# AdrianoEttari/DiffusionRemoteSensing

Measured on AMD Instinct MI355X. Metric: unet_denoise_steps_per_s, higher is better.
Workload: dtype f16 main + block-scaled fp6 (e2m3) cross terms of tap pairs on the wide 3x3 layers (FL, 11 of 11 launches of the dominant kernel); split bf16 x3 (hi + lo) everywhere else; f32 accumulate

## Files before the change

diffusionremotesensing_amd/csrc/resblock0_sp.hip:

```cpp
#include <stdio.h>
#include <stdlib.h>

#include "conv_epilogue.h"
#include "mfma_policy.h"
#include "sp_sync.h"

namespace {

constexpr int TW_ = 16, TH_ = 8, IW = TW_ + 2, IH = TH_ + 2, NPIX = IW * IH, NBLK_A = (NPIX + 15) / 16;
constexpr int IMG1 = 5 * 4 * 64 * 16, IMG2 = 36 * 32 * 16, IMGS = 4 * 32 * 16, WIN = NPIX * 128;
constexpr int NPOST = 16;
constexpr int XPLANE = (TH_ + 4) * (TW_ + 4) * 16 + 64, XT = 4 * XPLANE;

#ifdef DRS_SP_TIMELINE
__device__ unsigned long long drs_rb0_tl[32];
#define RB_STAMP(i) do { const unsigned long long t_ = __builtin_amdgcn_s_memtime(); tl[i] += t_ - tl_last; tl_last = t_; } while (0)
#else
#define RB_STAMP(i) do { } while (0)
#endif

__global__ __launch_bounds__(512, 1) void resblock0_kernel(ResBlock0Desc d, unsigned w1_gimage, unsigned w2_gimage,
                                                           unsigned ws_gimage) {
  extern __shared__ __attribute__((aligned(16))) char smem[];
  using P = PolicyBF16X3;
  using Frag = typename P::Frag;
  auto mfma = [](const bf16x8& w, const bf16x8& x, const f32x4& c) __attribute__((always_inline)) {
    return __builtin_amdgcn_mfma_f32_16x16x32_bf16(w, x, c, 0, 0, 0);
  };
  const int tid = threadIdx.x, lane = tid & 63, wave = __builtin_amdgcn_readfirstlane(tid >> 6);
  const int lr = lane & 15, kg = lane >> 4;
  char* sW1 = smem;
  char* sW2 = sW1 + 2 * IMG1;
  char* sWs = sW2 + 2 * IMG2;
  char* sWinAll = sWs + 2 * IMGS;
  char* sXAll = sWinAll + 2 * WIN;
  float* sB1 = reinterpret_cast<float*>(sXAll + 2 * XT);
  float* sB2 = sB1 + 64;
  unsigned* sCntRaw = reinterpret_cast<unsigned*>(sB2 + 32);
  float* sPost = sB2 + 32 + 8;
  const int npost = min(d.N, NPOST);
  {
    const char* w1 = reinterpret_cast<const char*>(d.w1);
    for (int i = tid; i < 2 * 20 * 64; i += 512) {
      const int im = i >= 20 * 64, idx = im ? i - 20 * 64 : i;
      const int ch = idx % 64, kgp = (idx / 64) & 3, j = idx / (4 * 64), tap = 2 * j + (kgp >> 1);
      u32x4 v = {0u, 0u, 0u, 0u};
      if (tap < 9) v = *reinterpret_cast<const u32x4*>(w1 + (size_t)im * w1_gimage + ((size_t)(tap * 4 + (kgp & 1)) * 64 + ch) * 16);
      *reinterpret_cast<u32x4*>(sW1 + (size_t)im * IMG1 + (size_t)idx * 16) = v;
    }
    auto copy = [&](char* dst, const char* src, int bytes) __attribute__((always_inline)) {
      for (int o = tid * 16; o < bytes; o += 512 * 16) *reinterpret_cast<u32x4*>(dst + o) = *reinterpret_cast<const u32x4*>(src + o);
    };
    const char* w2 = reinterpret_cast<const char*>(d.w2);
    const char* wsc = reinterpret_cast<const char*>(d.ws);
    copy(sW2, w2, IMG2);
    copy(sW2 + IMG2, w2 + w2_gimage, IMG2);
    copy(sWs, wsc, IMGS);
    copy(sWs + IMGS, wsc + ws_gimage, IMGS);
    for (int i = tid; i < 64; i += 512) sB1[i] = d.b1[i];
    for (int i = tid; i < 32; i += 512) sB2[i] = d.b2[i] + d.bs[i];
    if (tid < 8) sCntRaw[tid] = 0u;
    for (int i = tid; i < npost * 32; i += 512) sPost[i] = d.temb[(size_t)(i >> 5) * d.temb_cs + (i & 31)];
  }
  __syncthreads();

  const int grp = wave >> 2, gw = wave & 3;
  char* sWin = sWinAll + grp * WIN;
  const sp_flag_ptr cWritten = (sp_flag_ptr)(sCntRaw + 2 * grp), cRead = (sp_flag_ptr)(sCntRaw + 2 * grp + 1);
  const int gx = d.W / TW_, gy = d.H / TH_;
  const int total = d.N * gy * gx;
  const int xcd = blockIdx.x & 7, member = blockIdx.x >> 3, members = gridDim.x >> 3;
  const int t_lo = (int)((long long)total * xcd / 8), t_hi = (int)((long long)total * (xcd + 1) / 8);
  const char* zero = reinterpret_cast<const char*>(d.zero_line);
  const char* xb = reinterpret_cast<const char*>(d.x);
  char* sX = sXAll + grp * XT;
  const sp_flag_ptr cTile = (sp_flag_ptr)(sCntRaw + 4 + grp);
  constexpr int XPIX = (TH_ + 4) * (TW_ + 4), XW = TW_ + 4;
  int tx0 = 0, ty0 = 0, n = 0;
  const int qstep_ = 2 * (int)(gridDim.x >> 3);
  const int step_x = qstep_ % gx, step_y = (qstep_ / gx) % gy, step_n = qstep_ / (gx * gy);
  int bx = 0, by = 0;
  auto place_first = [&](int q) __attribute__((always_inline)) {
    bx = q % gx; by = (q / gx) % gy; n = q / (gx * gy);
    tx0 = bx * TW_; ty0 = by * TH_;
  };
  auto place_next = [&]() __attribute__((always_inline)) {
    bx += step_x;
    if (bx >= gx) { bx -= gx; ++by; }
    by += step_y;
    if (by >= gy) { by -= gy; ++n; }
    n += step_n;
    tx0 = bx * TW_; ty0 = by * TH_;
  };
  unsigned goff[4];
#pragma unroll
  for (int i = 0; i < 4; ++i) {
    const int e = i * 256 + gw * 64 + lane, pix = min(e >> 2, XPIX - 1);
    const int py = (pix * 3277) >> 16, px = pix - py * XW;
    goff[i] = (unsigned)((py * d.W + px) * 64 + (e & 3) * 16);
  }
  u32x4 xr[4];
  auto tile_load = [&]() __attribute__((always_inline)) {
    const char* ximg = xb + (size_t)n * d.H * d.W * 64;
    if (ty0 >= 2 && ty0 + TH_ + 2 <= d.H && tx0 >= 2 && tx0 + TW_ + 2 <= d.W) {
      typedef const __attribute__((address_space(1))) char* gptr;
      const unsigned long long gi = (unsigned long long)(ximg + ((long long)(ty0 - 2) * d.W + (tx0 - 2)) * 64);
      gptr g = (gptr)(((unsigned long long)(unsigned)__builtin_amdgcn_readfirstlane((int)(gi >> 32)) << 32) |
                      (unsigned)__builtin_amdgcn_readfirstlane((int)(unsigned)gi));
      asm volatile("" : "+s"(g));
#pragma unroll
      for (int i = 0; i < 4; ++i) xr[i] = *(const __attribute__((address_space(1))) u32x4*)(g + goff[i]);
    } else {
#pragma unroll
      for (int i = 0; i < 4; ++i) {
        const int e = i * 256 + gw * 64 + lane, pix = e >> 2;
        const int py = (pix * 3277) >> 16, px = pix - py * XW;
        const int y = ty0 - 2 + py, x = tx0 - 2 + px;
        const bool ok = pix < XPIX && y >= 0 && y < d.H && x >= 0 && x < d.W;
        xr[i] = *reinterpret_cast<const u32x4*>(ok ? ximg + ((size_t)y * d.W + x) * 64 + (e & 3) * 16 : zero);
      }
    }
  };
  auto tile_store = [&]() __attribute__((always_inline)) {
#pragma unroll
    for (int i = 0; i < 4; ++i) {
      const int e = i * 256 + gw * 64 + lane;
      if ((e >> 2) < XPIX) *reinterpret_cast<u32x4*>(sX + (e & 3) * XPLANE + (e >> 2) * 16) = xr[i];
    }
    sp_release(cTile, lane);
  };
  constexpr int MAXB = NBLK_A / 4;
  static_assert(MAXB * 4 == NBLK_A, "three blocks per wave");
  int wp[MAXB], relL[MAXB], tapL[5];
#pragma unroll
  for (int b = 0; b < MAXB; ++b) {
    const int p = min((gw + 4 * b) * 16 + lr, NPIX - 1);
    const int py = (p * 3641) >> 16, px = p - py * IW;
    wp[b] = p;
    relL[b] = ((py + 1) * XW + px + 1) * 16 + (kg & 1) * XPLANE;
  }
#pragma unroll
  for (int j = 0; j < 5; ++j) {
    const int tap = min(2 * j + (kg >> 1), 8);
    tapL[j] = ((tap / 3 - 1) * XW + tap % 3 - 1) * 16;
  }
  auto operand = [&](int b, int j) __attribute__((always_inline)) {
    const char* p = sX + relL[b] + tapL[j];
    return Frag{*reinterpret_cast<const bf16x8*>(p), *reinterpret_cast<const bf16x8*>(p + 2 * XPLANE)};
  };
  const int q0 = t_lo + 2 * member + grp, qstep = 2 * members;
#ifdef DRS_SP_TIMELINE
  unsigned long long tl[8] = {0, 0, 0, 0, 0, 0, 0, 0};
  const unsigned long long tl_begin = __builtin_amdgcn_s_memtime();
  unsigned long long tl_last = tl_begin, tl_n = 0;
#endif
  if (q0 < t_hi) {
    place_first(q0);
    tile_load();
    tile_store();
    if (q0 + qstep < t_hi) {
      place_next();
      tile_load();
      asm volatile("" :: "v"(xr[0]), "v"(xr[1]), "v"(xr[2]), "v"(xr[3]));
    }
  }
  if (grp == 1) { __builtin_amdgcn_s_sleep(64); __builtin_amdgcn_s_sleep(32); }
  unsigned k = 0;
  u32x4 kept[4] = {};
  int cbx = q0 % gx, cby = (q0 / gx) % gy, cn = q0 / (gx * gy);
  for (int q = q0; q < t_hi; q += qstep, ++k) {
#ifdef DRS_SP_TIMELINE
    ++tl_n;
#endif
    RB_STAMP(7);
    const int cty0 = cby * TH_, ctx0 = cbx * TW_;
    sp_poll_lds(cTile, 4u * (k + 1), d.fault);
    const bool more = q + qstep < t_hi;
    f32x4 acc[MAXB][4];
#pragma unroll
    for (int b = 0; b < MAXB; ++b)
#pragma unroll
      for (int t = 0; t < 4; ++t) acc[b][t] = f32x4{0.f, 0.f, 0.f, 0.f};
    const char* w1lane = sW1 + ((size_t)kg * 64 + lr) * 16;
    Frag a[2][MAXB], wfa[2][2];
#pragma unroll
    for (int b = 0; b < MAXB; ++b) a[0][b] = operand(b, 0);
#pragma unroll
    for (int u = 0; u < 2; ++u) wfa[0][u] = P::load(w1lane, (size_t)IMG1, (size_t)(u * 16) * 16);
#pragma unroll
    for (int st = 0; st < 10; ++st) {
      const int j = st >> 1, h = st & 1;
      if (st + 1 < 10) {
#pragma unroll
        for (int u = 0; u < 2; ++u)
          wfa[(st + 1) & 1][u] = P::load(w1lane, (size_t)IMG1, (size_t)(((st + 1) >> 1) * 4 * 64 + (((st + 1) & 1) * 2 + u) * 16) * 16);
      }
      if (h == 0 && j + 1 < 5) {
#pragma unroll
        for (int b = 0; b < MAXB; ++b) a[(j + 1) & 1][b] = operand(b, j + 1);
      }
      {
        const Frag (&wf)[2] = wfa[st & 1];
#pragma unroll
        for (int u = 0; u < 2; ++u)
#pragma unroll
          for (int b = 0; b < MAXB; ++b) acc[b][2 * h + u] = mfma(wf[u].lo, a[j & 1][b].hi, acc[b][2 * h + u]);
#pragma unroll
        for (int u = 0; u < 2; ++u)
#pragma unroll
          for (int b = 0; b < MAXB; ++b) acc[b][2 * h + u] = mfma(wf[u].hi, a[j & 1][b].lo, acc[b][2 * h + u]);
#pragma unroll
        for (int u = 0; u < 2; ++u)
#pragma unroll
          for (int b = 0; b < MAXB; ++b) acc[b][2 * h + u] = mfma(wf[u].hi, a[j & 1][b].hi, acc[b][2 * h + u]);
      }
      if (h == 0 && j + 1 < 5) __builtin_amdgcn_sched_group_barrier(0x100, 4 + 2 * MAXB, 0);
      else if (st + 1 < 10) __builtin_amdgcn_sched_group_barrier(0x100, 4, 0);
      __builtin_amdgcn_sched_group_barrier(0x008, 18, 0);
      __builtin_amdgcn_sched_barrier(0);
    }
    asm volatile("" :: "v"(kept[0]), "v"(kept[1]), "v"(kept[2]), "v"(kept[3]));
    RB_STAMP(0);
    Frag xs[2];
#pragma unroll
    for (int r = 0; r < 2; ++r) {
      const char* p = sX + ((2 + 2 * gw + r) * XW + 2 + lr) * 16 + (kg & 1) * XPLANE;
      xs[r] = Frag{*reinterpret_cast<const bf16x8*>(p), *reinterpret_cast<const bf16x8*>(p + 2 * XPLANE)};
    }
    float bm[8], bs[8], te[8];
    {
      const float4 m0 = *reinterpret_cast<const float4*>(sB1 + kg * 8), m1 = *reinterpret_cast<const float4*>(sB1 + kg * 8 + 4);
      const float4 s0 = *reinterpret_cast<const float4*>(sB1 + 32 + kg * 8), s1 = *reinterpret_cast<const float4*>(sB1 + 32 + kg * 8 + 4);
      float4 e0, e1;
      if (cn < npost) {
        e0 = *reinterpret_cast<const float4*>(sPost + cn * 32 + kg * 8); e1 = *reinterpret_cast<const float4*>(sPost + cn * 32 + kg * 8 + 4);
      } else {
        const float* gp = d.temb + (size_t)cn * d.temb_cs + kg * 8;
        e0 = *reinterpret_cast<const float4*>(gp); e1 = *reinterpret_cast<const float4*>(gp + 4);
      }
      bm[0] = m0.x; bm[1] = m0.y; bm[2] = m0.z; bm[3] = m0.w; bm[4] = m1.x; bm[5] = m1.y; bm[6] = m1.z; bm[7] = m1.w;
      bs[0] = s0.x; bs[1] = s0.y; bs[2] = s0.z; bs[3] = s0.w; bs[4] = s1.x; bs[5] = s1.y; bs[6] = s1.z; bs[7] = s1.w;
      te[0] = e0.x; te[1] = e0.y; te[2] = e0.z; te[3] = e0.w; te[4] = e1.x; te[5] = e1.y; te[6] = e1.z; te[7] = e1.w;
    }
    RB_STAMP(1);
    sp_poll_lds(cRead, 4u * k, d.fault);
    RB_STAMP(2);
#pragma unroll
    for (int b = 0; b < MAXB; ++b) {
      float v[8];
#pragma unroll
      for (int t = 0; t < 2; ++t)
#pragma unroll
        for (int i = 0; i < 4; ++i)
          v[t * 4 + i] = (drs_maxf(acc[b][t][i] + bm[t * 4 + i], 0.f) + (acc[b][t + 2][i] + bs[t * 4 + i])) + te[t * 4 + i];
      u32x4 hh, hl;
      drs_sp_split8(v, hh, hl);
      int p = wp[b];
      asm volatile("" : "+v"(p));
      const int py = (p * 3641) >> 16, px = p - py * IW;
      const int y = cty0 - 1 + py, x = ctx0 - 1 + px;
      const bool inside = y >= 0 && y < d.H && x >= 0 && x < d.W;
      if (!inside) { hh = u32x4{0u, 0u, 0u, 0u}; hl = u32x4{0u, 0u, 0u, 0u}; }
      if ((gw + 4 * b) * 16 + lr < NPIX) {
        char* wpix = sWin + p * 128;
        const int s0 = ((kg + p) & 7) * 16;
        *reinterpret_cast<u32x4*>(wpix + s0) = hh;
        *reinterpret_cast<u32x4*>(wpix + (s0 ^ 64)) = hl;
      }
    }
    sp_release(cWritten, lane);
    sp_poll_lds(cWritten, 4u * (k + 1), d.fault);
    if (more) tile_store();
    RB_STAMP(3);
    f32x4 o[2][2];
#pragma unroll
    for (int r = 0; r < 2; ++r)
#pragma unroll
      for (int t = 0; t < 2; ++t) o[r][t] = f32x4{0.f, 0.f, 0.f, 0.f};
    const char* w2lane = sW2 + ((size_t)kg * 32 + lr) * 16;
    auto win = [&](int row, int kx) __attribute__((always_inline)) {
      const int p = (2 * gw + row) * IW + lr + kx;
      const char* wpix = sWin + p * 128;
      const int s0 = ((kg + p) & 7) * 16;
      return Frag{*reinterpret_cast<const bf16x8*>(wpix + s0), *reinterpret_cast<const bf16x8*>(wpix + (s0 ^ 64))};
    };
    Frag wr_[4][3];
    auto win_row = [&](int row) __attribute__((always_inline)) {
#pragma unroll
      for (int kx = 0; kx < 3; ++kx) wr_[row][kx] = win(row, kx);
    };
    win_row(0);
    win_row(1);
    {
      const char* wslane = sWs + ((size_t)kg * 32 + lr) * 16;
      Frag wfb[2][2];
      wfb[0][0] = P::load(w2lane, (size_t)IMG2, 0);
      wfb[0][1] = P::load(w2lane, (size_t)IMG2, (size_t)16 * 16);
#pragma unroll
      for (int st = 0; st < 10; ++st) {
#pragma unroll
        for (int t = 0; t < 2; ++t) {
          if (st + 1 < 9) wfb[(st + 1) & 1][t] = P::load(w2lane, (size_t)IMG2, (size_t)((st + 1) * 4 * 32 + t * 16) * 16);
          else if (st + 1 < 10) wfb[(st + 1) & 1][t] = P::load(wslane, (size_t)IMGS, (size_t)(t * 16) * 16);
        }
        if (st == 0) win_row(2);
        if (st == 3) {
          win_row(3);
          sp_release(cRead, lane);
        }
        const int ky = st < 9 ? st / 3 : 0, kx = st < 9 ? st % 3 : 0;
        const Frag& x0f = st < 9 ? wr_[ky][kx] : xs[0];
        const Frag& x1f = st < 9 ? wr_[ky + 1][kx] : xs[1];
        const Frag (&wf)[2] = wfb[st & 1];
#pragma unroll
        for (int t = 0; t < 2; ++t) { o[0][t] = mfma(wf[t].lo, x0f.hi, o[0][t]); o[1][t] = mfma(wf[t].lo, x1f.hi, o[1][t]); }
#pragma unroll
        for (int t = 0; t < 2; ++t) { o[0][t] = mfma(wf[t].hi, x0f.lo, o[0][t]); o[1][t] = mfma(wf[t].hi, x1f.lo, o[1][t]); }
#pragma unroll
        for (int t = 0; t < 2; ++t) { o[0][t] = mfma(wf[t].hi, x0f.hi, o[0][t]); o[1][t] = mfma(wf[t].hi, x1f.hi, o[1][t]); }
        if (st == 0 || st == 3) __builtin_amdgcn_sched_group_barrier(0x100, 10, 0);
        else if (st + 1 < 10) __builtin_amdgcn_sched_group_barrier(0x100, 4, 0);
        __builtin_amdgcn_sched_group_barrier(0x008, 12, 0);
        __builtin_amdgcn_sched_barrier(0);
      }
    }
    if (q + 2 * qstep < t_hi) {
      place_next();
      tile_load();
    }
    RB_STAMP(4);
    {
      const float4 b0 = *reinterpret_cast<const float4*>(sB2 + kg * 8), b1 = *reinterpret_cast<const float4*>(sB2 + kg * 8 + 4);
      const float bb[8] = {b0.x, b0.y, b0.z, b0.w, b1.x, b1.y, b1.z, b1.w};
      const bool lo = lr < 8;
      const size_t pix0 = ((size_t)cn * d.H + cty0 + 2 * gw) * d.W + ctx0 + (lr & 7);
      char* g = reinterpret_cast<char*>(d.out) + pix0 * 128 + (lo ? 0 : 64) + kg * 16;
#pragma unroll
      for (int r = 0; r < 2; ++r) {
        float v[8];
#pragma unroll
        for (int i = 0; i < 4; ++i) { v[i] = drs_maxf(o[r][0][i] + bb[i], 0.f); v[4 + i] = drs_maxf(o[r][1][i] + bb[4 + i], 0.f); }
        u32x4 H, L;
        drs_sp_split8(v, H, L);
        const u32x4 got = drs_dpp_swap8(lo ? L : H);
        kept[2 * r] = lo ? H : got;
        kept[2 * r + 1] = lo ? got : L;
        char* gr = g + (size_t)r * d.W * 128;
        drs_store16(gr, kept[2 * r]);
        drs_store16(gr + 8 * 128, kept[2 * r + 1]);
      }
    }
    RB_STAMP(5);
    cbx += step_x;
    if (cbx >= gx) { cbx -= gx; ++cby; }
    cby += step_y;
    if (cby >= gy) { cby -= gy; ++cn; }
    cn += step_n;
  }
#ifdef DRS_SP_TIMELINE
  if (blockIdx.x == 0 && (wave == 0 || wave == 7) && lane == 0) {
    const int o = wave == 0 ? 0 : 16;
    for (int i = 0; i < 8; ++i) drs_rb0_tl[o + i] = tl[i];
    drs_rb0_tl[o + 8] = tl_n;
    drs_rb0_tl[o + 9] = __builtin_amdgcn_s_memtime() - tl_begin;
  }
#endif
}

size_t resblock0_lds(int N) { return (size_t)2 * (IMG1 + IMG2 + IMGS) + 2 * WIN + 2 * XT + (size_t)(64 + 32 + 8 + 32 * (N < NPOST ? N : NPOST)) * 4; }

}

bool drs_resblock0_supported(int Cin, int Cout, int H, int W) {
  static const bool env = !(getenv("DRS_RB0") && atoi(getenv("DRS_RB0")) == 0);
  return env && Cin == 16 && Cout == 32 && H >= 32 && W >= 32 && H % TH_ == 0 && W % TW_ == 0;
}

int drs_launch_resblock0(const ResBlock0Desc& d, hipStream_t s) {
  DRS_REQUIRE(drs_resblock0_supported(16, 32, d.H, d.W), DRS_ERR_SHAPE, "resblock0: H=%d W=%d", d.H, d.W);
  DRS_REQUIRE(d.x && d.w1 && d.b1 && d.temb && d.w2 && d.b2 && d.ws && d.bs && d.out && d.zero_line, DRS_ERR_ARG, "resblock0: null pointer");
  if (d.N == 0) return DRS_OK;
  int num_cu = 0;
  {
    const int rc = drs_kernel_prepare(reinterpret_cast<const void*>(resblock0_kernel), 160 * 1024, &num_cu);
    if (rc) return rc;
  }
  const unsigned w1_gimage = 9u * 4u * 64u * 16u, w2_gimage = 9u * 4u * 32u * 16u, ws_gimage = 4u * 32u * 16u;
  const int blocks = num_cu / 8 * 8;
  DRS_LAUNCH(resblock0_kernel, dim3((unsigned)blocks), dim3(512), resblock0_lds(d.N), s, d, w1_gimage, w2_gimage, ws_gimage);
  DRS_CHECK_HIP(hipGetLastError());
#ifdef DRS_SP_TIMELINE
  {
    unsigned long long h[32];
    hipEvent_t e0, e1;
    float ms = 0.f;
    DRS_CHECK_HIP(hipEventCreate(&e0)); DRS_CHECK_HIP(hipEventCreate(&e1));
    DRS_CHECK_HIP(hipEventRecord(e0, s));
    DRS_LAUNCH(resblock0_kernel, dim3((unsigned)blocks), dim3(512), resblock0_lds(d.N), s, d, w1_gimage, w2_gimage, ws_gimage);
    DRS_CHECK_HIP(hipEventRecord(e1, s));
    DRS_CHECK_HIP(hipStreamSynchronize(s));
    DRS_CHECK_HIP(hipEventElapsedTime(&ms, e0, e1));
    (void)hipEventDestroy(e0); (void)hipEventDestroy(e1);
    DRS_CHECK_HIP(hipMemcpyFromSymbol(h, HIP_SYMBOL(drs_rb0_tl), sizeof(h)));
    for (int w = 0; w < 2; ++w) {
      const unsigned long long* t = h + 16 * w;
      const double sc = t[8] ? 1.0 / (double)t[8] : 0.0;
      fprintf(stderr, "resblock0 %dx%d wave %d: %.1f us, %llu patches, alive %llu ticks (%.0f / patch) | top %.0f  A-mfma %.0f  A-epi %.0f  bar1 %.0f  "
              "winstore+bar2 %.0f  B-mfma %.0f  B-epi %.0f\n", d.H, d.W, w ? 7 : 0, ms * 1e3, t[8], t[9], t[9] * sc, t[7] * sc, t[0] * sc, t[1] * sc,
              t[2] * sc, t[3] * sc, t[4] * sc, t[5] * sc);
    }
  }
#endif
  return DRS_OK;
}
```

Before: 831.9.

## Overlap first tile loads with LDS weight fill and re-layout input planes

Restructures the resblock0 prologue so each lane issues all global loads for weights, biases and time embedding into registers before writing LDS. The first two input tiles are loaded before the weight fill so their latency overlaps it. Input-tile LDS planes are rearranged with a 64-byte offset on the hi/lo pair to shift bank mapping, and wave-to-group assignment is interleaved. The change also extends timeline instrumentation, and costs extra registers in the prologue.

Result: no change. 838.7 (median of 4 runs) (+0.8%).

```diff
diff --git a/diffusionremotesensing_amd/csrc/resblock0_sp.hip b/diffusionremotesensing_amd/csrc/resblock0_sp.hip
--- a/diffusionremotesensing_amd/csrc/resblock0_sp.hip
+++ b/diffusionremotesensing_amd/csrc/resblock0_sp.hip
@@ -10,10 +10,10 @@
 constexpr int TW_ = 16, TH_ = 8, IW = TW_ + 2, IH = TH_ + 2, NPIX = IW * IH, NBLK_A = (NPIX + 15) / 16;
 constexpr int IMG1 = 5 * 4 * 64 * 16, IMG2 = 36 * 32 * 16, IMGS = 4 * 32 * 16, WIN = NPIX * 128;
 constexpr int NPOST = 16;
-constexpr int XPLANE = (TH_ + 4) * (TW_ + 4) * 16 + 64, XT = 4 * XPLANE;
-
-#ifdef DRS_SP_TIMELINE
-__device__ unsigned long long drs_rb0_tl[32];
+constexpr int XPLANE = (TH_ + 4) * (TW_ + 4) * 16, XT = 4 * XPLANE + 256, XP1 = XPLANE, XP2 = 2 * XPLANE + 64;
+
+#ifdef DRS_SP_TIMELINE
+__device__ unsigned long long drs_rb0_tl[64];
 #define RB_STAMP(i) do { const unsigned long long t_ = __builtin_amdgcn_s_memtime(); tl[i] += t_ - tl_last; tl_last = t_; } while (0)
 #else
 #define RB_STAMP(i) do { } while (0)
@@ -39,32 +39,48 @@
   unsigned* sCntRaw = reinterpret_cast<unsigned*>(sB2 + 32);
   float* sPost = sB2 + 32 + 8;
   const int npost = min(d.N, NPOST);
-  {
+#ifdef DRS_SP_TIMELINE
+  const unsigned long long tl_entry = __builtin_amdgcn_s_memtime(), tl_rt_entry = __builtin_amdgcn_s_memrealtime();
+#endif
+  auto fill_lds = [&]() __attribute__((always_inline)) {
     const char* w1 = reinterpret_cast<const char*>(d.w1);
-    for (int i = tid; i < 2 * 20 * 64; i += 512) {
-      const int im = i >= 20 * 64, idx = im ? i - 20 * 64 : i;
-      const int ch = idx % 64, kgp = (idx / 64) & 3, j = idx / (4 * 64), tap = 2 * j + (kgp >> 1);
-      u32x4 v = {0u, 0u, 0u, 0u};
-      if (tap < 9) v = *reinterpret_cast<const u32x4*>(w1 + (size_t)im * w1_gimage + ((size_t)(tap * 4 + (kgp & 1)) * 64 + ch) * 16);
-      *reinterpret_cast<u32x4*>(sW1 + (size_t)im * IMG1 + (size_t)idx * 16) = v;
-    }
-    auto copy = [&](char* dst, const char* src, int bytes) __attribute__((always_inline)) {
-      for (int o = tid * 16; o < bytes; o += 512 * 16) *reinterpret_cast<u32x4*>(dst + o) = *reinterpret_cast<const u32x4*>(src + o);
-    };
     const char* w2 = reinterpret_cast<const char*>(d.w2);
     const char* wsc = reinterpret_cast<const char*>(d.ws);
-    copy(sW2, w2, IMG2);
-    copy(sW2 + IMG2, w2 + w2_gimage, IMG2);
-    copy(sWs, wsc, IMGS);
-    copy(sWs + IMGS, wsc + ws_gimage, IMGS);
-    for (int i = tid; i < 64; i += 512) sB1[i] = d.b1[i];
-    for (int i = tid; i < 32; i += 512) sB2[i] = d.b2[i] + d.bs[i];
+    constexpr int N1 = 2 * 20 * 64 / 512, P2 = IMG2 / 16, N2 = (2 * P2 + 511) / 512, PS = IMGS / 16;
+    static_assert(N1 * 512 == 2 * 20 * 64 && 2 * PS <= 512, "fill: pieces per lane");
+    u32x4 v1[N1], v2[N2], vs = {0u, 0u, 0u, 0u};
+#pragma unroll
+    for (int it = 0; it < N1; ++it) {
+      const int i = tid + it * 512, im = i >= 20 * 64, idx = im ? i - 20 * 64 : i;
+      const int ch = idx % 64, kgp = (idx / 64) & 3, j = idx / (4 * 64), tap = 2 * j + (kgp >> 1);
+      v1[it] = u32x4{0u, 0u, 0u, 0u};
+      if (tap < 9) v1[it] = *reinterpret_cast<const u32x4*>(w1 + (size_t)im * w1_gimage + ((size_t)(tap * 4 + (kgp & 1)) * 64 + ch) * 16);
+    }
+#pragma unroll
+    for (int it = 0; it < N2; ++it) {
+      const int i = tid + it * 512, im = i >= P2;
+      v2[it] = u32x4{0u, 0u, 0u, 0u};
+      if (i < 2 * P2) v2[it] = *reinterpret_cast<const u32x4*>(w2 + (size_t)im * w2_gimage + (size_t)(i - im * P2) * 16);
+    }
+    if (tid < 2 * PS) vs = *reinterpret_cast<const u32x4*>(wsc + (size_t)(tid >= PS) * ws_gimage + (size_t)(tid & (PS - 1)) * 16);
+    float fb1 = 0.f, fb2 = 0.f, fpost = 0.f;
+    if (tid < 64) fb1 = d.b1[tid];
+    if (tid < 32) fb2 = d.b2[tid] + d.bs[tid];
+    static_assert(NPOST * 32 <= 512, "fill: one time-embedding element per lane");
+    if (tid < npost * 32) fpost = d.temb[(size_t)(tid >> 5) * d.temb_cs + (tid & 31)];
+#pragma unroll
+    for (int it = 0; it < N1; ++it) *reinterpret_cast<u32x4*>(sW1 + (size_t)(tid + it * 512) * 16) = v1[it];
+#pragma unroll
+    for (int it = 0; it < N2; ++it)
+      if (tid + it * 512 < 2 * P2) *reinterpret_cast<u32x4*>(sW2 + (size_t)(tid + it * 512) * 16) = v2[it];
+    if (tid < 2 * PS) *reinterpret_cast<u32x4*>(sWs + (size_t)tid * 16) = vs;
+    if (tid < 64) sB1[tid] = fb1;
+    if (tid < 32) sB2[tid] = fb2;
     if (tid < 8) sCntRaw[tid] = 0u;
-    for (int i = tid; i < npost * 32; i += 512) sPost[i] = d.temb[(size_t)(i >> 5) * d.temb_cs + (i & 31)];
-  }
-  __syncthreads();
-
-  const int grp = wave >> 2, gw = wave & 3;
+    if (tid < npost * 32) sPost[tid] = fpost;
+  };
+
+  const int grp = ((wave >> 2) ^ (wave >> 1)) & 1, gw = (wave - 2 * grp) & 3;
   char* sWin = sWinAll + grp * WIN;
   const sp_flag_ptr cWritten = (sp_flag_ptr)(sCntRaw + 2 * grp), cRead = (sp_flag_ptr)(sCntRaw + 2 * grp + 1);
   const int gx = d.W / TW_, gy = d.H / TH_;
@@ -100,7 +116,7 @@
     goff[i] = (unsigned)((py * d.W + px) * 64 + (e & 3) * 16);
   }
   u32x4 xr[4];
-  auto tile_load = [&]() __attribute__((always_inline)) {
+  auto tile_load = [&](u32x4 (&xr)[4]) __attribute__((always_inline)) {
     const char* ximg = xb + (size_t)n * d.H * d.W * 64;
     if (ty0 >= 2 && ty0 + TH_ + 2 <= d.H && tx0 >= 2 && tx0 + TW_ + 2 <= d.W) {
       typedef const __attribute__((address_space(1))) char* gptr;
@@ -121,11 +137,11 @@
       }
     }
   };
-  auto tile_store = [&]() __attribute__((always_inline)) {
+  auto tile_store = [&](const u32x4 (&xr)[4]) __attribute__((always_inline)) {
 #pragma unroll
     for (int i = 0; i < 4; ++i) {
       const int e = i * 256 + gw * 64 + lane;
-      if ((e >> 2) < XPIX) *reinterpret_cast<u32x4*>(sX + (e & 3) * XPLANE + (e >> 2) * 16) = xr[i];
+      if ((e >> 2) < XPIX) *reinterpret_cast<u32x4*>(sX + (e & 1) * XP1 + ((e >> 1) & 1) * XP2 + (e >> 2) * 16) = xr[i];
     }
     sp_release(cTile, lane);
   };
@@ -137,7 +153,7 @@
     const int p = min((gw + 4 * b) * 16 + lr, NPIX - 1);
     const int py = (p * 3641) >> 16, px = p - py * IW;
     wp[b] = p;
-    relL[b] = ((py + 1) * XW + px + 1) * 16 + (kg & 1) * XPLANE;
+    relL[b] = ((py + 1) * XW + px + 1) * 16 + (kg & 1) * XP1;
   }
 #pragma unroll
   for (int j = 0; j < 5; ++j) {
@@ -146,24 +162,31 @@
   }
   auto operand = [&](int b, int j) __attribute__((always_inline)) {
     const char* p = sX + relL[b] + tapL[j];
-    return Frag{*reinterpret_cast<const bf16x8*>(p), *reinterpret_cast<const bf16x8*>(p + 2 * XPLANE)};
+    return Frag{*reinterpret_cast<const bf16x8*>(p), *reinterpret_cast<const bf16x8*>(p + XP2)};
   };
   const int q0 = t_lo + 2 * member + grp, qstep = 2 * members;
-#ifdef DRS_SP_TIMELINE
-  unsigned long long tl[8] = {0, 0, 0, 0, 0, 0, 0, 0};
-  const unsigned long long tl_begin = __builtin_amdgcn_s_memtime();
+  {
+    u32x4 x1st[4] = {};
+    if (q0 < t_hi) {
+      place_first(q0);
+      tile_load(x1st);
+      if (q0 + qstep < t_hi) {
+        place_next();
+        tile_load(xr);
+      }
+    }
+    fill_lds();
+    __syncthreads();
+    if (q0 < t_hi) tile_store(x1st);
+  }
+  if (q0 + qstep < t_hi) {
+    asm volatile("" :: "v"(xr[0]), "v"(xr[1]), "v"(xr[2]), "v"(xr[3]));
+  }
+#ifdef DRS_SP_TIMELINE
+  unsigned long long tl[16] = {0, 0, 0, 0, 0, 0, 0, 0, 0, 0, 0, 0, 0, 0, 0, 0};
+  const unsigned long long tl_begin = __builtin_amdgcn_s_memtime(), tl_prologue = tl_begin - tl_entry;
   unsigned long long tl_last = tl_begin, tl_n = 0;
 #endif
-  if (q0 < t_hi) {
-    place_first(q0);
-    tile_load();
-    tile_store();
-    if (q0 + qstep < t_hi) {
-      place_next();
-      tile_load();
-      asm volatile("" :: "v"(xr[0]), "v"(xr[1]), "v"(xr[2]), "v"(xr[3]));
-    }
-  }
   if (grp == 1) { __builtin_amdgcn_s_sleep(64); __builtin_amdgcn_s_sleep(32); }
   unsigned k = 0;
   u32x4 kept[4] = {};
@@ -224,8 +247,8 @@
     Frag xs[2];
 #pragma unroll
     for (int r = 0; r < 2; ++r) {
-      const char* p = sX + ((2 + 2 * gw + r) * XW + 2 + lr) * 16 + (kg & 1) * XPLANE;
-      xs[r] = Frag{*reinterpret_cast<const bf16x8*>(p), *reinterpret_cast<const bf16x8*>(p + 2 * XPLANE)};
+      const char* p = sX + ((2 + 2 * gw + r) * XW + 2 + lr) * 16 + (kg & 1) * XP1;
+      xs[r] = Frag{*reinterpret_cast<const bf16x8*>(p), *reinterpret_cast<const bf16x8*>(p + XP2)};
     }
     float bm[8], bs[8], te[8];
     {
@@ -269,9 +292,11 @@
       }
     }
     sp_release(cWritten, lane);
+    RB_STAMP(3);
     sp_poll_lds(cWritten, 4u * (k + 1), d.fault);
-    if (more) tile_store();
-    RB_STAMP(3);
+    RB_STAMP(6);
+    if (more) tile_store(xr);
+    RB_STAMP(8);
     f32x4 o[2][2];
 #pragma unroll
     for (int r = 0; r < 2; ++r)
@@ -326,7 +351,7 @@
     }
     if (q + 2 * qstep < t_hi) {
       place_next();
-      tile_load();
+      tile_load(xr);
     }
     RB_STAMP(4);
     {
@@ -359,10 +384,14 @@
   }
 #ifdef DRS_SP_TIMELINE
   if (blockIdx.x == 0 && (wave == 0 || wave == 7) && lane == 0) {
-    const int o = wave == 0 ? 0 : 16;
-    for (int i = 0; i < 8; ++i) drs_rb0_tl[o + i] = tl[i];
-    drs_rb0_tl[o + 8] = tl_n;
-    drs_rb0_tl[o + 9] = __builtin_amdgcn_s_memtime() - tl_begin;
+    const int o = wave == 0 ? 0 : 32;
+    const unsigned long long t_end = __builtin_amdgcn_s_memtime();
+    for (int i = 0; i < 16; ++i) drs_rb0_tl[o + i] = tl[i];
+    drs_rb0_tl[o + 16] = tl_n;
+    drs_rb0_tl[o + 17] = t_end - tl_begin;
+    drs_rb0_tl[o + 18] = tl_prologue;
+    drs_rb0_tl[o + 19] = __builtin_amdgcn_s_memrealtime() - tl_rt_entry;
+    drs_rb0_tl[o + 20] = t_end - tl_entry;
   }
 #endif
 }
@@ -391,7 +420,7 @@
   DRS_CHECK_HIP(hipGetLastError());
 #ifdef DRS_SP_TIMELINE
   {
-    unsigned long long h[32];
+    unsigned long long h[64];
     hipEvent_t e0, e1;
     float ms = 0.f;
     DRS_CHECK_HIP(hipEventCreate(&e0)); DRS_CHECK_HIP(hipEventCreate(&e1));
@@ -403,11 +432,12 @@
     (void)hipEventDestroy(e0); (void)hipEventDestroy(e1);
     DRS_CHECK_HIP(hipMemcpyFromSymbol(h, HIP_SYMBOL(drs_rb0_tl), sizeof(h)));
     for (int w = 0; w < 2; ++w) {
-      const unsigned long long* t = h + 16 * w;
-      const double sc = t[8] ? 1.0 / (double)t[8] : 0.0;
-      fprintf(stderr, "resblock0 %dx%d wave %d: %.1f us, %llu patches, alive %llu ticks (%.0f / patch) | top %.0f  A-mfma %.0f  A-epi %.0f  bar1 %.0f  "
-              "winstore+bar2 %.0f  B-mfma %.0f  B-epi %.0f\n", d.H, d.W, w ? 7 : 0, ms * 1e3, t[8], t[9], t[9] * sc, t[7] * sc, t[0] * sc, t[1] * sc,
-              t[2] * sc, t[3] * sc, t[4] * sc, t[5] * sc);
+      const unsigned long long* t = h + 32 * w;
+      const double sc = t[16] ? 1.0 / (double)t[16] : 0.0;
+      fprintf(stderr, "resblock0 %dx%d wave %d: %.1f us, %llu patches, alive %llu ticks (%.0f / patch), prologue %llu, in kernel %llu ticks = %.1f us "
+              "(%.0f MHz) | top %.0f  A-mfma %.0f  A-epi %.0f  bar1 %.0f  winstore %.0f  bar2 %.0f  tilestore %.0f  B-mfma %.0f  B-epi %.0f\n",
+              d.H, d.W, w ? 7 : 0, ms * 1e3, t[16], t[17], t[17] * sc, t[18], t[20], t[19] * 0.01, t[19] ? t[20] / (t[19] * 0.01) : 0.0,
+              t[7] * sc, t[0] * sc, t[1] * sc, t[2] * sc, t[3] * sc, t[6] * sc, t[8] * sc, t[4] * sc, t[5] * sc);
     }
   }
 #endif
```
